# QZ1-boy/CDFO

Hardware: NVIDIA B200
Metric: HR frames/sec, 1080p x4 LD-QP37 (higher is better)
Workload: dtype bf16

## Files before the change

cdfo_b200/_lib.py:

```python
import ctypes
import os
import re
import weakref

import torch

_HERE = os.path.dirname(os.path.abspath(__file__))
SO_PATH = os.path.join(_HERE, "libcdfo_b200.so")

OK = 0
F32, F16, BF16 = 0, 1, 2
_DTYPES = {torch.float32: F32, torch.float16: F16, torch.bfloat16: BF16}


class CdfoError(RuntimeError):
    pass


_lib = None
HEADER = os.path.join(os.path.dirname(_HERE), "include", "cdfo_b200.h")


def _ctype(decl):
    d = decl.strip()
    if "*" in d:
        return ctypes.c_void_p
    base = re.sub(r"\b(const|unsigned|signed)\b", "", d).split()
    t = base[0] if base else "int"
    return {"float": ctypes.c_float, "double": ctypes.c_double, "size_t": ctypes.c_size_t, "int": ctypes.c_int, "int64_t": ctypes.c_int64,
            "uint8_t": ctypes.c_uint8, "long": ctypes.c_long}.get(t, ctypes.c_int)


def prototypes(header=HEADER):
    src = re.sub(r"/\*.*?\*/", "", open(header).read(), flags=re.S)
    src = re.sub(r"//[^\n]*", "", src)
    out = {}
    for ret, name, params in re.findall(r"\b(const\s+char\s*\*|size_t|int|void)\s*(cdfo_[a-z0-9_]+)\s*\(([^)]*)\)\s*;", src, flags=re.S):
        params = " ".join(params.split())
        args = [] if params in ("", "void") else [_ctype(a) for a in params.split(",")]
        res = ctypes.c_char_p if "char" in ret else (ctypes.c_size_t if ret == "size_t" else (None if ret == "void" else ctypes.c_int))
        out[name] = (res, args)
    return out


def _bind_prototypes(handle):
    if not os.path.isfile(HEADER):
        raise CdfoError("cdfo_b200: %s not found (the ctypes prototypes are taken from it)" % HEADER)
    for name, (res, args) in prototypes().items():
        fn = getattr(handle, name, None)
        if fn is None:
            raise CdfoError("cdfo_b200: %s declares %s but %s does not export it (stale build?)" % (HEADER, name, SO_PATH))
        fn.restype, fn.argtypes = res, args


def lib():
    global _lib
    if _lib is None:
        if not os.path.isfile(SO_PATH):
            raise CdfoError(
                "cdfo_b200: %s not found -- build it with `python cdfo_b200/csrc/build.py` "
                "(there is no CPU or PyTorch fallback for this path)" % SO_PATH)
        _lib = ctypes.CDLL(SO_PATH)
        _bind_prototypes(_lib)
    return _lib


_LAUNCHES = {"cdfo_mv_end_fix": 3, "cdfo_lra_fwd": 5, "cdfo_lra_c8_fwd": 5, "cdfo_mdta_fwd": 3, "cdfo_mdta_c8_fwd": 3, "cdfo_psnr_ssim_u8": 3,
             "cdfo_lra_mask_logits_fwd": 2,
             "cdfo_spatial_gate_c8_fwd": 2}
launch_count = 0


def call(name, *args):
    global launch_count
    rc = getattr(lib(), name)(*args)
    if rc != OK:
        check(rc, name)
    launch_count += _LAUNCHES.get(name, 1)
    return rc


def check(rc, what=""):
    if rc != OK:
        msg = lib().cdfo_last_error().decode("utf-8", "replace")
        raise CdfoError("%s failed (status %d): %s" % (what or "cdfo call", rc, msg))


def dtype_code(t: torch.Tensor) -> int:
    try:
        return _DTYPES[t.dtype]
    except KeyError:
        raise CdfoError("cdfo_b200: unsupported dtype %s" % t.dtype)


def ptr(t):
    return ctypes.c_void_p(0 if t is None else t.data_ptr())


def stream_ptr(device=None):
    return ctypes.c_void_p(torch.cuda.current_stream(device).cuda_stream)


def require_cuda(*tensors):
    for t in tensors:
        if t is not None and not t.is_cuda:
            raise NotImplementedError("cdfo_b200 ops are CUDA-only (got a %s tensor)" % t.device)


class TensorCache:

    def __init__(self):
        self._d = {}

    def get(self, t, build, kind=None):
        key = (id(t), kind)
        sig = (t.data_ptr(), str(t.device), t._version, t.dtype)
        hit = self._d.get(key)
        if hit is not None and hit[0]() is t and hit[1] == sig:
            return hit[2]
        val = build()
        d = self._d
        self._d[key] = (weakref.ref(t, lambda _r, k=key: d.pop(k, None)), sig, val)
        return val

    def __len__(self):
        return len(self._d)
```

cdfo_b200/csrc/lra.cu:

```cuda
#include <cuda.h>
#include <cstring>

#include "cdfo_common.cuh"
#include "sm100_ptx.cuh"

namespace cdfo {

__device__ __forceinline__ float warp_max(float v) {
#pragma unroll
  for (int o = 16; o > 0; o >>= 1) v = fmaxf(v, __shfl_xor_sync(0xffffffffu, v, o));
  return v;
}
__device__ __forceinline__ float warp_sum(float v) {
#pragma unroll
  for (int o = 16; o > 0; o >>= 1) v += __shfl_xor_sync(0xffffffffu, v, o);
  return v;
}

__global__ void lra_mask_kernel(const float *__restrict__ u, const float *__restrict__ vmax, const float *__restrict__ qv,
                                uint8_t *__restrict__ midx, float *__restrict__ qsel, int HW) {
  __shared__ float vm[64];
  const int b = blockIdx.y;
  if (threadIdx.x < 64) vm[threadIdx.x] = vmax[b * 64 + threadIdx.x];
  __syncthreads();
// ... 391 lines not shown
  }
}

constexpr int kColWarps = 9, kColThreads = kColWarps * 32;

__global__ void __launch_bounds__(kColThreads, 1) lra_col_kernel(const float *__restrict__ vrow_t, const uint8_t *__restrict__ midx,
                                                                const float *__restrict__ qsel, float *__restrict__ long_out,
                                                                LraTables t, int H, int W) {
  extern __shared__ __align__(16) float sm[];
  const int b = blockIdx.y, w = blockIdx.x;
  const int HW = H * W;
  const int Hk = (H + 63) & ~63;
  float *Q = sm;
  float *V = Q + Hk * kLd;
  float *sq = V;
  const int tid = threadIdx.x, lane = tid & 31, warp = tid >> 5, g = lane >> 2, tq = lane & 3;
  float kh[9];
#pragma unroll
  for (int i = 0; i < 9; ++i) kh[i] = t.kh[i];

  for (int e = tid; e < (H + 8) * 64; e += kColThreads) {
    const int h = (e >> 6) - 4, c = e & 63;
    float v = 0.f;
    if (h >= 0 && h < H) {
      v = t.beta;
      const int cm = midx[(size_t)b * HW + h * W + w];
      if (cm != 255) {
        const int ti = cm - c + 4;
        if (ti >= 0 && ti <= 8) v = fmaf(__ldg(t.kw + ti), qsel[(size_t)b * HW + h * W + w], v);
      }
    }
    sq[e] = v;
  }
  __syncthreads();
  for (int e = tid; e < Hk * 64; e += kColThreads) {
    const int h = e >> 6, c = e & 63;
    float acc = 0.f;
    if (h < H) {
      acc = t.bh;
#pragma unroll
      for (int i = 0; i < 9; ++i) acc = fmaf(kh[i], sq[(h + i) * 64 + c], acc);
    }
    Q[h * kLd + c] = __uint_as_float(to_tf32(acc));
  }
  __syncthreads();
  const float *vsrc = vrow_t + ((size_t)b * W + w) * H * 64;
  for (int e = tid; e < Hk * 16; e += kColThreads) {
    const int r = e >> 4, c4 = (e & 15) * 4;
    float4 v = make_float4(0.f, 0.f, 0.f, 0.f);
    if (r < H) v = *reinterpret_cast<const float4 *>(vsrc + (size_t)r * 64 + c4);
    v.x = __uint_as_float(to_tf32(v.x)); v.y = __uint_as_float(to_tf32(v.y));
    v.z = __uint_as_float(to_tf32(v.z)); v.w = __uint_as_float(to_tf32(v.w));
    *reinterpret_cast<float4 *>(V + r * kLd + c4) = v;
  }
  __syncthreads();

  const uint32_t *Qu = reinterpret_cast<const uint32_t *>(Q), *Vu = reinterpret_cast<const uint32_t *>(V);
  const int n_qt = (H + 15) >> 4, n_kb = Hk >> 6;
  for (int qt = warp; qt < n_qt; qt += kColWarps) {
    const int q0 = qt * 16;
    uint32_t aq[8][4];
#pragma unroll
    for (int s = 0; s < 8; ++s) {
      aq[s][0] = Qu[(q0 + g) * kLd + 8 * s + tq];
      aq[s][1] = Qu[(q0 + g + 8) * kLd + 8 * s + tq];
      aq[s][2] = Qu[(q0 + g) * kLd + 8 * s + tq + 4];
      aq[s][3] = Qu[(q0 + g + 8) * kLd + 8 * s + tq + 4];
    }
    float o[8][4];
#pragma unroll
    for (int n = 0; n < 8; ++n)
#pragma unroll
      for (int i = 0; i < 4; ++i) o[n][i] = 0.f;
    float m_run[2] = {-INFINITY, -INFINITY}, l_run[2] = {0.f, 0.f};
    for (int kb = 0; kb < n_kb; ++kb) {
      const int key0 = kb * 64;
      float sc[8][4];
#pragma unroll
      for (int n = 0; n < 8; ++n) {
#pragma unroll
        for (int i = 0; i < 4; ++i) sc[n][i] = 0.f;
        const uint32_t *kr = Qu + (key0 + 8 * n + g) * kLd + tq;
#pragma unroll
        for (int s = 0; s < 8; ++s) mma_tf32(sc[n], aq[s], kr[8 * s], kr[8 * s + 4]);
      }
      flash_tile_block(sc, m_run, l_run, o, Vu, key0, H, g, tq);
    }
#pragma unroll
    for (int r = 0; r < 2; ++r) {
      l_run[r] += __shfl_xor_sync(0xffffffffu, l_run[r], 1);
      l_run[r] += __shfl_xor_sync(0xffffffffu, l_run[r], 2);
    }
    const float inv0 = 1.f / l_run[0], inv1 = 1.f / l_run[1];
    const int h0 = q0 + g, h1 = q0 + g + 8;
#pragma unroll
    for (int n = 0; n < 8; ++n) {
      if (h0 < H) *reinterpret_cast<float2 *>(long_out + (((size_t)b * H + h0) * W + w) * 64 + 8 * n + 2 * tq) = make_float2(o[n][0] * inv0, o[n][1] * inv0);
      if (h1 < H) *reinterpret_cast<float2 *>(long_out + (((size_t)b * H + h1) * W + w) * 64 + 8 * n + 2 * tq) = make_float2(o[n][2] * inv1, o[n][3] * inv1);
    }
  }
}

constexpr int kQw = 36;

__device__ __forceinline__ void mma_bf16(float (&d)[4], const uint32_t (&a)[4], uint32_t b0, uint32_t b1) {
  asm volatile("mma.sync.aligned.m16n8k16.row.col.f32.bf16.bf16.f32 {%0, %1, %2, %3}, {%4, %5, %6, %7}, {%8, %9}, {%0, %1, %2, %3};"
               : "+f"(d[0]), "+f"(d[1]), "+f"(d[2]), "+f"(d[3])
               : "r"(a[0]), "r"(a[1]), "r"(a[2]), "r"(a[3]), "r"(b0), "r"(b1));
}
__device__ __forceinline__ uint32_t pack_bf16x2(float lo, float hi) {
  __nv_bfloat162 v = __floats2bfloat162_rn(lo, hi);
  return *reinterpret_cast<uint32_t *>(&v);
}

__global__ void __launch_bounds__(kColThreads, 2) lra_col_bf16_kernel(const float *__restrict__ vrow_t, const uint8_t *__restrict__ midx,
                                                                     const float *__restrict__ qsel, float *__restrict__ long_out,
                                                                     LraTables t, int H, int W) {
  extern __shared__ __align__(16) uint32_t smu[];
  const int b = blockIdx.y, w = blockIdx.x;
  const int HW = H * W;
  const int Hk = (H + 63) & ~63;
  const int SW = Hk / 2 + 4;
  uint32_t *Qw = smu;
  uint32_t *Vt = Qw + Hk * kQw;
  float *cq = reinterpret_cast<float *>(Vt + 64 * SW);
  int *cm = reinterpret_cast<int *>(cq + H + 8);
  float *kws = reinterpret_cast<float *>(cm + H + 8);
  const int tid = threadIdx.x, lane = tid & 31, warp = tid >> 5, g = lane >> 2, tq = lane & 3;
  float kh[9];
#pragma unroll
  for (int i = 0; i < 9; ++i) kh[i] = t.kh[i];
  if (tid < 9) kws[tid] = t.kw[tid];
  for (int e = tid; e < H + 8; e += kColThreads) {
    const int h = e - 4;
    int c = -1;
    float q = 0.f;
    if (h >= 0 && h < H) {
      c = midx[(size_t)b * HW + h * W + w];
      q = qsel[(size_t)b * HW + h * W + w];
    }
    cm[e] = c;
    cq[e] = q;
  }
  {
    const float *vsrc = vrow_t + ((size_t)b * W + w) * H * 64;
    for (int e = tid; e < (Hk / 2) * 16; e += kColThreads) {
      const int kp = (e >> 6) * 4 + (e & 3), c4 = (e >> 2) & 15;
      float4 v0 = make_float4(0.f, 0.f, 0.f, 0.f), v1 = v0;
      if (2 * kp < H) v0 = __ldg(reinterpret_cast<const float4 *>(vsrc + (size_t)(2 * kp) * 64 + c4 * 4));
      if (2 * kp + 1 < H) v1 = __ldg(reinterpret_cast<const float4 *>(vsrc + (size_t)(2 * kp + 1) * 64 + c4 * 4));
      const uint32_t wv[4] = {pack_bf16x2(v0.x, v1.x), pack_bf16x2(v0.y, v1.y), pack_bf16x2(v0.z, v1.z), pack_bf16x2(v0.w, v1.w)};
#pragma unroll
      for (int i = 0; i < 4; ++i) {
        const int j = (i + (c4 >> 1)) & 3;
        Vt[(c4 * 4 + j) * SW + kp] = j == 0 ? wv[0] : (j == 1 ? wv[1] : (j == 2 ? wv[2] : wv[3]));
      }
    }
  }
  __syncthreads();
  for (int e = tid; e < Hk * 32; e += kColThreads) {
    const int h = e >> 5, c0 = (e & 31) * 2;
    float a0 = 0.f, a1 = 0.f;
    if (h < H) {
      a0 = a1 = t.bh;
#pragma unroll
      for (int i = 0; i < 9; ++i) {
        const int c = cm[h + i];
        if (c < 0) continue;
        float s0 = t.beta, s1 = t.beta;
        if (c != 255) {
          const int t0 = c - c0 + 4, t1 = t0 - 1;
          const float q = cq[h + i];
          if (t0 >= 0 && t0 <= 8) s0 = fmaf(kws[t0], q, s0);
          if (t1 >= 0 && t1 <= 8) s1 = fmaf(kws[t1], q, s1);
        }
        a0 = fmaf(kh[i], s0, a0);
        a1 = fmaf(kh[i], s1, a1);
      }
    }
    Qw[h * kQw + (e & 31)] = pack_bf16x2(a0, a1);
  }
  __syncthreads();

  const int n_qt = (H + 15) >> 4, n_kb = Hk >> 6;
  for (int qt = warp; qt < n_qt; qt += kColWarps) {
    const int q0 = qt * 16;
    float o[8][4];
#pragma unroll
    for (int n = 0; n < 8; ++n)
#pragma unroll
      for (int i = 0; i < 4; ++i) o[n][i] = 0.f;
    float m_run[2] = {-INFINITY, -INFINITY}, l_run[2] = {0.f, 0.f};
    for (int kb = 0; kb < n_kb; ++kb) {
      const int key0 = kb * 64;
      float sc[8][4];
      {
        uint32_t aq[4][4];
#pragma unroll
        for (int s = 0; s < 4; ++s) {
          aq[s][0] = Qw[(q0 + g) * kQw + 8 * s + tq];
          aq[s][1] = Qw[(q0 + g + 8) * kQw + 8 * s + tq];
          aq[s][2] = Qw[(q0 + g) * kQw + 8 * s + tq + 4];
          aq[s][3] = Qw[(q0 + g + 8) * kQw + 8 * s + tq + 4];
        }
#pragma unroll
        for (int n = 0; n < 8; ++n) {
#pragma unroll
          for (int i = 0; i < 4; ++i) sc[n][i] = 0.f;
          const uint32_t *kr = Qw + (key0 + 8 * n + g) * kQw + tq;
#pragma unroll
          for (int s = 0; s < 4; ++s) mma_bf16(sc[n], aq[s], kr[8 * s], kr[8 * s + 4]);
        }
      }
      float mx[2] = {-INFINITY, -INFINITY};
#pragma unroll
      for (int n = 0; n < 8; ++n) {
        const int key = key0 + 8 * n + 2 * tq;
        if (key >= H) { sc[n][0] = -INFINITY; sc[n][2] = -INFINITY; }
        if (key + 1 >= H) { sc[n][1] = -INFINITY; sc[n][3] = -INFINITY; }
        mx[0] = fmaxf(mx[0], fmaxf(sc[n][0], sc[n][1]));
        mx[1] = fmaxf(mx[1], fmaxf(sc[n][2], sc[n][3]));
      }
      float scale[2];
#pragma unroll
      for (int r = 0; r < 2; ++r) {
        mx[r] = fmaxf(mx[r], __shfl_xor_sync(0xffffffffu, mx[r], 1));
        mx[r] = fmaxf(mx[r], __shfl_xor_sync(0xffffffffu, mx[r], 2));
        const float m_new = fmaxf(m_run[r], mx[r]);
        scale[r] = expf(m_run[r] - m_new);
        m_run[r] = m_new;
        l_run[r] *= scale[r];
      }
#pragma unroll
      for (int n = 0; n < 8; ++n) {
        sc[n][0] = expf(sc[n][0] - m_run[0]); sc[n][1] = expf(sc[n][1] - m_run[0]);
        sc[n][2] = expf(sc[n][2] - m_run[1]); sc[n][3] = expf(sc[n][3] - m_run[1]);
        l_run[0] += sc[n][0] + sc[n][1];
        l_run[1] += sc[n][2] + sc[n][3];
        o[n][0] *= scale[0]; o[n][1] *= scale[0]; o[n][2] *= scale[1]; o[n][3] *= scale[1];
      }
#pragma unroll
      for (int s = 0; s < 4; ++s) {
        const uint32_t ap[4] = {pack_bf16x2(sc[2 * s][0], sc[2 * s][1]), pack_bf16x2(sc[2 * s][2], sc[2 * s][3]),
                                pack_bf16x2(sc[2 * s + 1][0], sc[2 * s + 1][1]), pack_bf16x2(sc[2 * s + 1][2], sc[2 * s + 1][3])};
        const uint32_t *vr = Vt + g * SW + (key0 >> 1) + 8 * s + tq;
#pragma unroll
        for (int n = 0; n < 8; ++n) mma_bf16(o[n], ap, vr[8 * n * SW], vr[8 * n * SW + 4]);
      }
    }
#pragma unroll
    for (int r = 0; r < 2; ++r) {
      l_run[r] += __shfl_xor_sync(0xffffffffu, l_run[r], 1);
      l_run[r] += __shfl_xor_sync(0xffffffffu, l_run[r], 2);
    }
    const float inv0 = 1.f / l_run[0], inv1 = 1.f / l_run[1];
    const int h0 = q0 + g, h1 = q0 + g + 8;
#pragma unroll
    for (int n = 0; n < 8; ++n) {
      if (h0 < H) *reinterpret_cast<float2 *>(long_out + (((size_t)b * H + h0) * W + w) * 64 + 8 * n + 2 * tq) = make_float2(o[n][0] * inv0, o[n][1] * inv0);
      if (h1 < H) *reinterpret_cast<float2 *>(long_out + (((size_t)b * H + h1) * W + w) * 64 + 8 * n + 2 * tq) = make_float2(o[n][2] * inv1, o[n][3] * inv1);
    }
  }
}

constexpr int kWinThreads = 256;
__global__ void __launch_bounds__(kWinThreads) lra_win_kernel(const float *__restrict__ qv, const uint8_t *__restrict__ midx,
                                                             float *__restrict__ loc_out, int H, int W) {
  extern __shared__ __align__(16) float sm[];
  float *q = sm;
  float *v = q + 64 * kLd;
  float *Ps = v + 64 * kLd;
  const int b = blockIdx.z, wy = blockIdx.y, wx = blockIdx.x;
  const int HW = H * W;
  const int tid = threadIdx.x;
  static_assert(kWinThreads == 256, "one token and 16 + 16 channels per thread");
  {
    const int tok = tid & 63, cg = tid >> 6;
    const int h = wy * 8 + (tok >> 3), w = wx * 8 + (tok & 7);
    const size_t pix = (size_t)h * W + w;
    const int cm = midx[(size_t)b * HW + pix];
    const float *qp = qv + ((size_t)b * 128 + cg) * HW + pix;
    float qr[16], vv[16];
#pragma unroll
    for (int k = 0; k < 16; ++k) {
      qr[k] = __ldg(qp + (size_t)(4 * k) * HW);
      vv[k] = __ldg(qp + (size_t)(64 + 4 * k) * HW);
    }
#pragma unroll
    for (int k = 0; k < 16; ++k) {
      const int c = 4 * k + cg;
      q[tok * kLd + c] = cm == c ? 0.f : qr[k];
      v[tok * kLd + c] = vv[k];
    }
  }
  __syncthreads();
  const float *Kcur = q;
  flash_block_fp32_kptr(q, &Kcur, v, Ps, 64, [&](int) {}, [&](int tok, int c4, float4 val) {
    const int h = wy * 8 + (tok >> 3), w = wx * 8 + (tok & 7);
    *reinterpret_cast<float4 *>(loc_out + (((size_t)b * H + h) * W + w) * 64 + c4) = val;
  });
}

constexpr int kWinTcThreads = 128, kWinLd = 36;
__global__ void __launch_bounds__(kWinTcThreads, 6) lra_win_tc_kernel(const float *__restrict__ qv, const uint8_t *__restrict__ midx,
                                                                      float *__restrict__ loc_out, int H, int W) {
  __shared__ uint32_t Qh[64 * kWinLd], Ql[64 * kWinLd], Vt[64 * kWinLd], Vl[64 * kWinLd];
  const int b = blockIdx.z, wy = blockIdx.y, wx = blockIdx.x;
  const int HW = H * W;
  const int tid = threadIdx.x, lane = tid & 31, warp = tid >> 5, g = lane >> 2, tq = lane & 3;
  {
    const int tok = tid & 63, half = tid >> 6;
    const int h = wy * 8 + (tok >> 3), w = wx * 8 + (tok & 7);
    const size_t pix = (size_t)h * W + w;
    const int cm = midx[(size_t)b * HW + pix];
    const float *qp = qv + ((size_t)b * 128 + half * 32) * HW + pix;
#pragma unroll 4
    for (int k = 0; k < 16; ++k) {
      const int c = half * 32 + 2 * k;
      float q0 = __ldg(qp + (size_t)(2 * k) * HW), q1 = __ldg(qp + (size_t)(2 * k + 1) * HW);
      if (cm == c) q0 = 0.f;
      if (cm == c + 1) q1 = 0.f;
      const __nv_bfloat16 h0 = __float2bfloat16_rn(q0), h1 = __float2bfloat16_rn(q1);
      Qh[tok * kWinLd + (c >> 1)] = pack_bf16x2(__bfloat162float(h0), __bfloat162float(h1));
      Ql[tok * kWinLd + (c >> 1)] = pack_bf16x2(q0 - __bfloat162float(h0), q1 - __bfloat162float(h1));
      const float v0 = __ldg(qp + (size_t)(64 + 2 * k) * HW), v1 = __ldg(qp + (size_t)(64 + 2 * k + 1) * HW);
      const __nv_bfloat16 vh0 = __float2bfloat16_rn(v0), vh1 = __float2bfloat16_rn(v1);
      reinterpret_cast<__nv_bfloat16 *>(Vt)[(c * kWinLd) * 2 + tok] = vh0;
      reinterpret_cast<__nv_bfloat16 *>(Vt)[((c + 1) * kWinLd) * 2 + tok] = vh1;
      reinterpret_cast<__nv_bfloat16 *>(Vl)[(c * kWinLd) * 2 + tok] = __float2bfloat16_rn(v0 - __bfloat162float(vh0));
      reinterpret_cast<__nv_bfloat16 *>(Vl)[((c + 1) * kWinLd) * 2 + tok] = __float2bfloat16_rn(v1 - __bfloat162float(vh1));
    }
  }
  __syncthreads();
  const int q0r = warp * 16;
  uint32_t ah[4][4], al[4][4];
#pragma unroll
  for (int s = 0; s < 4; ++s) {
    ah[s][0] = Qh[(q0r + g) * kWinLd + 8 * s + tq];      ah[s][1] = Qh[(q0r + g + 8) * kWinLd + 8 * s + tq];
    ah[s][2] = Qh[(q0r + g) * kWinLd + 8 * s + tq + 4];  ah[s][3] = Qh[(q0r + g + 8) * kWinLd + 8 * s + tq + 4];
    al[s][0] = Ql[(q0r + g) * kWinLd + 8 * s + tq];      al[s][1] = Ql[(q0r + g + 8) * kWinLd + 8 * s + tq];
    al[s][2] = Ql[(q0r + g) * kWinLd + 8 * s + tq + 4];  al[s][3] = Ql[(q0r + g + 8) * kWinLd + 8 * s + tq + 4];
  }
  float sc[8][4];
#pragma unroll
  for (int n = 0; n < 8; ++n) {
#pragma unroll
    for (int i = 0; i < 4; ++i) sc[n][i] = 0.f;
    const uint32_t *kh_ = Qh + (8 * n + g) * kWinLd + tq, *kl_ = Ql + (8 * n + g) * kWinLd + tq;
#pragma unroll
    for (int s = 0; s < 4; ++s) {
      const uint32_t bh0 = kh_[8 * s], bh1 = kh_[8 * s + 4];
      mma_bf16(sc[n], al[s], bh0, bh1);
      mma_bf16(sc[n], ah[s], kl_[8 * s], kl_[8 * s + 4]);
      mma_bf16(sc[n], ah[s], bh0, bh1);
    }
  }
  float mx[2] = {-INFINITY, -INFINITY}, sum[2] = {0.f, 0.f};
#pragma unroll
  for (int n = 0; n < 8; ++n) {
    mx[0] = fmaxf(mx[0], fmaxf(sc[n][0], sc[n][1]));
    mx[1] = fmaxf(mx[1], fmaxf(sc[n][2], sc[n][3]));
  }
#pragma unroll
  for (int r = 0; r < 2; ++r) {
    mx[r] = fmaxf(mx[r], __shfl_xor_sync(0xffffffffu, mx[r], 1));
    mx[r] = fmaxf(mx[r], __shfl_xor_sync(0xffffffffu, mx[r], 2));
  }
#pragma unroll
  for (int n = 0; n < 8; ++n) {
    sc[n][0] = expf(sc[n][0] - mx[0]); sc[n][1] = expf(sc[n][1] - mx[0]);
    sc[n][2] = expf(sc[n][2] - mx[1]); sc[n][3] = expf(sc[n][3] - mx[1]);
    sum[0] += sc[n][0] + sc[n][1];
    sum[1] += sc[n][2] + sc[n][3];
  }
  float o[8][4];
#pragma unroll
  for (int n = 0; n < 8; ++n)
#pragma unroll
    for (int i = 0; i < 4; ++i) o[n][i] = 0.f;
#pragma unroll
  for (int s = 0; s < 4; ++s) {
    uint32_t ap[4], apl[4];
#pragma unroll
    for (int i = 0; i < 4; ++i) {
      const float p0 = sc[2 * s + (i >> 1)][2 * (i & 1)], p1 = sc[2 * s + (i >> 1)][2 * (i & 1) + 1];
      const float h0 = __bfloat162float(__float2bfloat16_rn(p0)), h1 = __bfloat162float(__float2bfloat16_rn(p1));
      ap[i] = pack_bf16x2(h0, h1);
      apl[i] = pack_bf16x2(p0 - h0, p1 - h1);
    }
    const uint32_t *vr = Vt + g * kWinLd + 8 * s + tq, *vl = Vl + g * kWinLd + 8 * s + tq;
#pragma unroll
    for (int n = 0; n < 8; ++n) {
      const uint32_t b0 = vr[8 * n * kWinLd], b1 = vr[8 * n * kWinLd + 4];
      mma_bf16(o[n], apl, b0, b1);
      mma_bf16(o[n], ap, vl[8 * n * kWinLd], vl[8 * n * kWinLd + 4]);
      mma_bf16(o[n], ap, b0, b1);
    }
  }
#pragma unroll
  for (int r = 0; r < 2; ++r) {
    sum[r] += __shfl_xor_sync(0xffffffffu, sum[r], 1);
    sum[r] += __shfl_xor_sync(0xffffffffu, sum[r], 2);
  }
  const float inv0 = 1.f / sum[0], inv1 = 1.f / sum[1];
  const int t0 = q0r + g, t1 = t0 + 8;
  float *d0 = loc_out + (((size_t)b * H + wy * 8 + (t0 >> 3)) * W + wx * 8 + (t0 & 7)) * 64 + 2 * tq;
  float *d1 = loc_out + (((size_t)b * H + wy * 8 + (t1 >> 3)) * W + wx * 8 + (t1 & 7)) * 64 + 2 * tq;
#pragma unroll
  for (int n = 0; n < 8; ++n) {
    *reinterpret_cast<float2 *>(d0 + 8 * n) = make_float2(o[n][0] * inv0, o[n][1] * inv0);
    *reinterpret_cast<float2 *>(d1 + 8 * n) = make_float2(o[n][2] * inv1, o[n][3] * inv1);
  }
}

}

using namespace cdfo;

typedef CUresult (*LraEncodeTiledFn)(CUtensorMap *, CUtensorMapDataType, cuuint32_t, void *, const cuuint64_t *, const cuuint64_t *,
                                     const cuuint32_t *, const cuuint32_t *, CUtensorMapInterleave, CUtensorMapSwizzle,
                                     CUtensorMapL2promotion, CUtensorMapFloatOOBfill);
static LraEncodeTiledFn lra_encode_tiled_fn() {
  static LraEncodeTiledFn fn = nullptr;
  if (!fn) {
    void *ptr = nullptr;
    cudaDriverEntryPointQueryResult q;
    if (cudaGetDriverEntryPoint("cuTensorMapEncodeTiled", &ptr, cudaEnableDefault, &q) == cudaSuccess && q == cudaDriverEntryPointSuccess)
      fn = reinterpret_cast<LraEncodeTiledFn>(ptr);
  }
  return fn;
}

static bool g_lra_row_tma = true;
extern "C" int cdfo_lra_set_row_tma(int on) {
  g_lra_row_tma = on != 0;
  return CDFO_OK;
}
static bool g_lra_col_tf32 = false;
static bool g_lra_col_tc = true;
static bool g_lra_win_tc = true;
extern "C" int cdfo_lra_set_col_precision(int tf32) {
  g_lra_col_tf32 = tf32 != 0;
  return CDFO_OK;
}
extern "C" int cdfo_lra_set_col_tcgen05(int on) {
  g_lra_col_tc = on != 0;
  return CDFO_OK;
}
extern "C" int cdfo_lra_set_win_tensor_core(int on) {
  g_lra_win_tc = on != 0;
  return CDFO_OK;
}

extern "C" size_t cdfo_lra_workspace_bytes(int B, int H, int W) {
  const size_t P = (size_t)B * H * W;
  return P * (1 + 4) + 3 * P * 64 * 4 + 256;
}

static int lra_run(const float *qv, const float *u, const float *vmax, const float *x, const float *x2, const float *tables,
                   float beta, float bh, const float *fuse_w, const float *fuse_b, float *out, void *out_c8, int out_channels,
                   int channel0, void *workspace, int B, int H, int W, void *stream);

extern "C" int cdfo_lra_fwd(const float *qv, const float *u, const float *vmax, const float *x, const float *x2, const float *tables,
                            float beta, float bh, const float *fuse_w, const float *fuse_b, float *out, void *workspace, int B,
                            int H, int W, void *stream) {
  return lra_run(qv, u, vmax, x, x2, tables, beta, bh, fuse_w, fuse_b, out, nullptr, 0, 0, workspace, B, H, W, stream);
}

extern "C" int cdfo_lra_c8_fwd(const float *qv, const float *u, const float *vmax, const float *x, const float *x2, const float *tables,
                               float beta, float bh, const float *fuse_w, const float *fuse_b, void *out_c8, int out_channels,
                               int channel0, void *workspace, int B, int H, int W, void *stream) {
  CDFO_REQUIRE(out_c8 && ((uintptr_t)out_c8 & 15) == 0, CDFO_ERR_NULL, "cdfo_lra_c8_fwd: out_c8 must be a 16-byte aligned pointer");
  CDFO_REQUIRE(out_channels % 8 == 0 && channel0 % 8 == 0 && channel0 >= 0 && channel0 + 64 <= out_channels, CDFO_ERR_SHAPE,
               "cdfo_lra_c8_fwd: channels [%d, %d) do not fit %d output channels (multiples of 8)", channel0, channel0 + 64, out_channels);
  return lra_run(qv, u, vmax, x, x2, tables, beta, bh, fuse_w, fuse_b, nullptr, out_c8, out_channels, channel0, workspace, B, H, W, stream);
}

static int lra_run(const float *qv, const float *u, const float *vmax, const float *x, const float *x2, const float *tables,
                   float beta, float bh, const float *fuse_w, const float *fuse_b, float *out, void *out_c8, int out_channels,
                   int channel0, void *workspace, int B, int H, int W, void *stream) {
  CDFO_REQUIRE(qv && u && vmax && x && tables && fuse_w && fuse_b && (out || out_c8) && workspace, CDFO_ERR_NULL, "cdfo_lra_fwd: NULL pointer");
  CDFO_REQUIRE(B > 0 && B <= 65535 && H > 0 && W > 0 && H % 8 == 0 && W % 8 == 0, CDFO_ERR_SHAPE,
               "cdfo_lra_fwd: H and W must be multiples of the window size 8 (got %d x %d)", H, W);
  cudaStream_t s = (cudaStream_t)stream;
  const size_t P = (size_t)B * H * W;
  const int HW = H * W;
  uint8_t *ws = (uint8_t *)workspace;
  float *qsel = (float *)ws;
  float *vrow_t = qsel + P;
  float *long_out = vrow_t + P * 64;
  float *loc_out = long_out + P * 64;
  uint8_t *midx = (uint8_t *)(loc_out + P * 64);
  LraTables t{tables, tables + 9, tables + 18, tables + 82, beta, bh};

  lra_mask_kernel<<<dim3(ceil_div(HW, 128), B), 128, 0, s>>>(u, vmax, qv, midx, qsel, HW);

  const int Wk = (W + 63) & ~63;
  const size_t row_smem = ((size_t)Wk * kLd + 4096 + 3 * (size_t)Wk + 64 + kRowThreads + 2 * (size_t)Wk) * 4;
  const int Hk = (H + 63) & ~63;
  const size_t col_v = (size_t)Hk * kLd > (size_t)(H + 8) * 64 ? (size_t)Hk * kLd : (size_t)(H + 8) * 64;
  const size_t col_smem = ((size_t)Hk * kLd + col_v) * 4;
  const size_t win_smem = (size_t)3 * 64 * kLd * 4;
  const int kDynMax = 224 * 1024;
  CDFO_REQUIRE(row_smem <= (size_t)kDynMax && col_smem <= (size_t)kDynMax, CDFO_ERR_UNSUPPORTED,
               "cdfo_lra_fwd: frame %d x %d exceeds the shared-memory row/column buffers (W <= 704, H <= 384)", H, W);
  static bool attr = false;
  if (!attr) {
    cudaError_t e1 = cudaFuncSetAttribute(lra_row_kernel<false>, cudaFuncAttributeMaxDynamicSharedMemorySize, kDynMax);
    if (e1 == cudaSuccess) e1 = cudaFuncSetAttribute(lra_row_kernel<true>, cudaFuncAttributeMaxDynamicSharedMemorySize, kDynMax);
    cudaError_t e2 = cudaFuncSetAttribute(lra_col_kernel, cudaFuncAttributeMaxDynamicSharedMemorySize, kDynMax);
    if (e2 == cudaSuccess) e2 = cudaFuncSetAttribute(lra_col_bf16_kernel, cudaFuncAttributeMaxDynamicSharedMemorySize, kDynMax);
    cudaError_t e3 = cudaFuncSetAttribute(lra_win_kernel, cudaFuncAttributeMaxDynamicSharedMemorySize, (int)win_smem);
    if (e1 != cudaSuccess || e2 != cudaSuccess || e3 != cudaSuccess)
      return fail(CDFO_ERR_CUDA, "cdfo_lra_fwd: cudaFuncSetAttribute failed: %s", cudaGetErrorString(e1 != cudaSuccess ? e1 : (e2 != cudaSuccess ? e2 : e3)));
    attr = true;
  }
  {
    CUtensorMap qm;
    memset(&qm, 0, sizeof(qm));
    bool row_tma = g_lra_row_tma && W % 4 == 0 && ((uintptr_t)qv & 15) == 0 && row_smem + kRowRawBytes <= (size_t)kDynMax;
    if (row_tma) {
      static LraEncodeTiledFn enc = lra_encode_tiled_fn();
      if (enc) {
        const cuuint64_t gdim[3] = {(cuuint64_t)W, (cuuint64_t)H, (cuuint64_t)B * 128};
        const cuuint64_t gstr[2] = {(cuuint64_t)W * 4, (cuuint64_t)H * W * 4};
        const cuuint32_t box[3] = {kRowPiece, 1, 64};
        const cuuint32_t estr[3] = {1, 1, 1};
        CUresult cr = enc(&qm, CU_TENSOR_MAP_DATA_TYPE_FLOAT32, 3, const_cast<float *>(qv), gdim, gstr, box, estr, CU_TENSOR_MAP_INTERLEAVE_NONE,
                          CU_TENSOR_MAP_SWIZZLE_NONE, CU_TENSOR_MAP_L2_PROMOTION_L2_128B, CU_TENSOR_MAP_FLOAT_OOB_FILL_NONE);
        CDFO_REQUIRE(cr == CUDA_SUCCESS, CDFO_ERR_CUDA, "cuTensorMapEncodeTiled(qv rows) failed with CUresult %d", (int)cr);
      } else {
        row_tma = false;
      }
    }
    if (row_tma) lra_row_kernel<true><<<dim3(H, B), kRowThreads, row_smem + kRowRawBytes, s>>>(qm, qv, midx, qsel, vrow_t, t, H, W);
    else lra_row_kernel<false><<<dim3(H, B), kRowThreads, row_smem, s>>>(qm, qv, midx, qsel, vrow_t, t, H, W);
  }
  int col_done = 0;
  if (!g_lra_col_tf32 && g_lra_col_tc) {
    col_done = lra_col_sm100_launch(vrow_t, midx, qsel, long_out, t, B, H, W, s);
    if (col_done < 0) return col_done;
  }
  if (col_done) {
  } else if (g_lra_col_tf32) {
    lra_col_kernel<<<dim3(W, B), kColThreads, col_smem, s>>>(vrow_t, midx, qsel, long_out, t, H, W);
  } else {
    const size_t col16_smem = ((size_t)Hk * kQw + 64 * ((size_t)Hk / 2 + 4) + 2 * (size_t)(H + 8) + 16) * 4;
    lra_col_bf16_kernel<<<dim3(W, B), kColThreads, col16_smem, s>>>(vrow_t, midx, qsel, long_out, t, H, W);
  }
  if (g_lra_win_tc) lra_win_tc_kernel<<<dim3(W / 8, H / 8, B), kWinTcThreads, 0, s>>>(qv, midx, loc_out, H, W);
  else lra_win_kernel<<<dim3(W / 8, H / 8, B), kWinThreads, win_smem, s>>>(qv, midx, loc_out, H, W);
  if (int rc = check_launch("cdfo_lra_fwd")) return rc;
  return pointwise_conv(long_out, loc_out, fuse_w, fuse_b, x, x2, out, B, 128, 64, HW, 0, 1, s, out_c8, out_channels, channel0);
}
```

include/cdfo_b200.h:

```cpp
#ifndef CDFO_B200_H_
#define CDFO_B200_H_

#include <stddef.h>
#include <stdint.h>

#ifdef __cplusplus
extern "C" {
#endif

typedef enum cdfo_status {
  CDFO_OK = 0,
  CDFO_ERR_SHAPE = -1,
  CDFO_ERR_NULL = -2,
  CDFO_ERR_CUDA = -3,
  CDFO_ERR_UNSUPPORTED = -4,
  CDFO_ERR_NO_DEVICE = -5
} cdfo_status;

typedef enum cdfo_dtype { CDFO_F32 = 0, CDFO_F16 = 1, CDFO_BF16 = 2 } cdfo_dtype;
#define CDFO_FIELDS_F16X4 16

const char *cdfo_last_error(void);
int cdfo_version(void);
int cdfo_device_ok(int dev);

int cdfo_dcn_fwd(const void *x, const void *offset, const void *mask, const void *weight,
                 const void *bias, void *y, int B, int C, int H, int W, int Co, int kh, int kw,
                 int stride_h, int stride_w, int pad_h, int pad_w, int dil_h, int dil_w,
                 int groups, int dg, int dtype, void *stream);

int cdfo_dcn_sample_index(const float *offset, int32_t *idx, int B, int H, int W, int kh, int kw,
                          int stride_h, int stride_w, int pad_h, int pad_w, int dil_h, int dil_w,
                          int dg, void *stream);

int cdfo_flow_warp_fwd(const float *x, const float *flow, float *y, int B, int C, int H, int W,
                       int32_t *idx, void *stream);

int cdfo_mv2mvs(const void *mv, int mv_is_int32, float *flows, int H, int W, void *stream);
int cdfo_mv2mvs_ra(const void *mv_l0, const void *mv_l1, int mv_is_int32, float *flows, int H, int W, void *stream);
int cdfo_mv_end_fix(float *flows, int B, int H, int W, int i, int max_idx, void *stream);

int cdfo_prior_conv_fwd(const float *x, const float *w, const float *bias, float *y, int B, int Co, int H, int W, void *stream);
int cdfo_prior_conv_act_fwd(const float *x, const float *w, const float *bias, float *y, int B, int Co, int H, int W, int relu, void *stream);

int cdfo_pack_c8(const float *x_nchw, void *x_c8, int B, int C, int H, int W, void *stream);
int cdfo_pack_c8_into(const float *x_nchw, void *x_c8, int B, int C, int H, int W, int out_channels, int channel0, void *stream);
int cdfo_unpack_c8(const void *x_c8, float *x_nchw, int B, int C, int H, int W, void *stream);

int cdfo_dcn_sm100_fwd(const void *x_q4p, const void *offset, const void *mask, const float *mv,
                       const void *wpk, const float *bias, void *y, int B, int H, int W, int dg,
                       int off_dtype, int out_mode, int num_ctas, int x_batch, long long off_bstride,
                       long long msk_bstride, void *stream);
int cdfo_dcn_sm100_pack_weight(const float *w, void *wpk, void *stream);
int cdfo_pack_q4p(const float *x_nchw, void *x_q4p, int B, int C, int H, int W, void *stream);
int cdfo_dcn_tex_sm100_fwd(const void *x_q4t, const void *fields, const float *mv, const void *wpk, const float *bias,
                           void *y, int B, int H, int W, int dg, int out_mode, int num_ctas, int x_batch,
                           long long fields_bstride, void *stream);
int cdfo_dcn_tex_sm100_set_fields_path(int use_tma);
int cdfo_dcn_tex_sm100_stacked_fwd(const void *x_q4t, const void *fields, const float *mv, const void *wpk, const float *bias,
                                   void *y_stack, int n_seq, int n_groups, int stack_chunks, const int *group_chunk, int H,
                                   int W, int dg, int x_batch, void *stream);
int cdfo_dcn_tex_sm100_pack_weight(const float *w, void *wpk, void *stream);
int cdfo_mv_head_dcn_fused_sm100_fwd(const void *z_c8, const void *head_wpk, const float *head_bias, float magnitude,
                                     const void *x_q4t, const float *mv, const void *dcn_wpk, const float *dcn_bias, void *y,
                                     void *fields_out, int B, int H, int W, int out_mode, int x_batch, int num_ctas, void *stream);
int cdfo_mv_head_dcn_fused_sm100_stacked_fwd(const void *z_c8, const void *head_wpk, const float *head_bias, float magnitude,
                                             const void *x_q4t, const float *mv, const void *dcn_wpk, const float *dcn_bias,
                                             void *y_stack, int n_seq, int n_groups, int stack_chunks, const int *group_chunk,
                                             int H, int W, int x_batch, void *stream);
int cdfo_pack_q4t(const float *x_nchw, void *x_q4t, int B, int C, int H, int W, void *stream);
int cdfo_q4t_pitch(int W);
size_t cdfo_q4t_bytes(int B, int C, int H, int W);
int cdfo_conv3x3_sm100_fwd(const void *x_c8, const void *wpk, const float *bias, const void *resid_c8, void *y,
                           int B, int Cin, int Cout, int H, int W, int act, int out_mode, void *stream);
int cdfo_mv_offset_head_sm100_fwd(const void *z_c8, const void *wpk, const float *bias, const void *first, void *out,
                                  int B, int Cin, int dg, int H, int W, float magnitude, void *stream);
int cdfo_mv_offset_head_dual_sm100_fwd(const void *z_c8, const void *wpk, const float *bias, void *out, int B, int Cin, int dg, int H,
                                       int W, float magnitude, void *stream);
int cdfo_conv_last_skip_sm100_fwd(const void *x_c8, const void *wpk, const float *bias, const float *lr, float *y, int B,
                                  int Cin, int H, int W, void *stream);
int cdfo_conv3x3_sm100_pack_weight(const float *w, void *wpk, int Cout, int Cin, void *stream);
int cdfo_conv_sm100_fwd(const void *x_c8, const void *wpk, const float *bias, const void *resid_c8, void *y, int B, int Cin,
                        int Cout, int H, int W, int ksize, int act, int out_mode, void *stream);
int cdfo_conv_sm100_pack_weight(const float *w, void *wpk, int Cout, int Cin, int ksize, void *stream);
size_t cdfo_conv_sm100_weight_bytes(int Cout, int Cin, int ksize);
size_t cdfo_conv3x3_sm100_weight_bytes(int Cout, int Cin);
int cdfo_conv3x3_sm100_ntile(int Cout, int Cin);
int cdfo_mdta_fwd(const float *x, int x_batch, const float *extra, const float *pred, const float *flow,
                  const float *fusion_w, const float *du_w1, const float *du_b1, const float *du_w2, const float *du_b2,
                  const float *temperature, const float *proj_w, int heads, int mode, void *out, float *ca_sums,
                  void *workspace, int B, int H, int W, void *stream);
int cdfo_mdta_c8_fwd(const void *x_c8, int x_batch, const void *extra_c8, const void *pred_c8, const float *flow, const float *fusion_w,
                     const float *du_w1, const float *du_b1, const float *du_w2, const float *du_b2, const float *temperature,
                     const float *proj_w, int heads, void *out_c8, void *workspace, int B, int H, int W, void *stream);
size_t cdfo_mdta_workspace_bytes(int B, int H, int W, int heads);
int cdfo_mdta_parts(int B);
int cdfo_channel_gate_fwd(const float *partial_sums, int parts, const float *w1, const float *b1, const float *w2,
                          const float *b2, float *gate, int B, int C, int Cmid, int HW, void *stream);
int cdfo_pack_c8_scaled(const float *x_nchw, const float *scale, void *x_c8, int B, int C, int H, int W, void *stream);
int cdfo_unpack_c8_add(const void *x_c8, const float *add_nchw, int add_batch, float *y_nchw, int B, int C, int H, int W,
                       void *stream);
int cdfo_resample_c8(const void *a, const void *b, const void *base, void *y, int B, int C, int Ho, int Wo, int mode, void *stream);
int cdfo_lra_fwd(const float *qv, const float *u, const float *vmax, const float *x, const float *x2, const float *tables,
                 float beta, float bh, const float *fuse_w, const float *fuse_b, float *out, void *workspace, int B, int H, int W,
                 void *stream);
int cdfo_lra_set_col_precision(int tf32);
int cdfo_lra_set_col_tcgen05(int on);
int cdfo_lra_set_win_tensor_core(int on);
int cdfo_lra_set_row_tma(int on);
int cdfo_lra_c8_fwd(const float *qv, const float *u, const float *vmax, const float *x, const float *x2, const float *tables,
                    float beta, float bh, const float *fuse_w, const float *fuse_b, void *out_c8, int out_channels, int channel0,
                    void *workspace, int B, int H, int W, void *stream);
int cdfo_pointwise_conv_fwd(const float *in1, const float *in2, const float *w, const float *bias, const float *resid1,
                            const float *resid2, float *out, int B, int K, int Co, int H, int W, int act, int mode, void *stream);
int cdfo_pointwise_conv_c8_fwd(const float *in1, const float *in2, const float *w, const float *bias, const float *resid1,
                               const float *resid2, void *out_c8, int B, int K, int Co, int H, int W, int act, int mode,
                               int out_channels, int channel0, void *stream);
size_t cdfo_lra_workspace_bytes(int B, int H, int W);
int cdfo_layernorm_c_fwd(const void *x, const float *gamma, const float *beta, void *y, int B, int C, int H, int W, float eps,
                         int dtype, void *stream);
int cdfo_dwconv3x3_fwd(const void *x, const float *w, void *y, int B, int C, int H, int W, int dtype, void *stream);
int cdfo_mdta_gram_fwd(const void *qk, float *partial, int B, int Ctot, int H, int W, int parts, int dtype, void *stream);
int cdfo_conv3x3_pair_sm100_supported(int Cout, int Cin);
size_t cdfo_conv3x3_pair_sm100_weight_bytes(int Cout, int Cin);
int cdfo_conv3x3_pair_sm100_pack_weight(const float *w, void *wpk, int Cout, int Cin, void *stream);
int cdfo_conv3x3_pair_sm100_fwd(const void *x_c8, const void *wpk, const float *bias, const void *resid_c8, void *y_c8, int B, int Cin,
                                int Cout, int H, int W, int act, void *stream);
int cdfo_conv3x3_pair_sm100_planes_fwd(const void *x_c8, const void *wpk, const float *bias, const void *resid_c8, void *y, int B,
                                       int Cin, int Cout, int H, int W, int act, int y_planes, void *stream);
int cdfo_conv3x3_pair_sm100_edge_fwd(const void *x_c8, const void *wpk, const float *bias, const float *bias_edge, const void *resid_c8,
                                     void *y, int B, int Cin, int Cout, int H, int W, int act, int y_planes, void *stream);
int cdfo_conv4x4s2_pair_sm100_supported(int Cout, int Cin);
size_t cdfo_conv4x4s2_pair_sm100_weight_bytes(int Cin);
int cdfo_conv4x4s2_pair_sm100_pack_weight(const float *w3, void *wpk, int Cin, void *stream);
int cdfo_conv4x4s2_pair_sm100_fwd(const void *x_c8, const void *wpk, const float *bias, const void *resid_c8, void *y_c8, int B, int Cin,
                                  int H_in, int W_in, void *stream);
int cdfo_conv4x4s2_pair_sm100_planes_fwd(const void *x, const void *wpk, const float *bias, const void *resid_c8, void *y_c8, int B,
                                         int Cin, int H_in, int W_in, int x_planes, void *stream);
int cdfo_conv4x4s2_pair_sm100_block_fwd(const void *x, const void *wpk, const float *bias, const void *resid_c8, const void *up_c8,
                                        void *y_c8, void *half_c8, int B, int Cin, int H_in, int W_in, int x_planes, void *stream);
int cdfo_planes_to_unit_f32(const void *src, int src_kind, float *dst, int n_planes, int H_in, int W, int H_out, void *stream);
int cdfo_sr_to_u8(const float *sr, uint8_t *out, int n_planes, int H_in, int W, int H_out, void *stream);
size_t cdfo_psnr_ssim_workspace_bytes(int B, int H, int W, int border);
int cdfo_psnr_ssim_u8(const uint8_t *res, const uint8_t *gt, int B, int H, int W, int border, double *frame_out, double *accum,
                      void *workspace, void *stream);
int cdfo_umma_selftest(const void *A, const void *B, float *D, int swap_lbo_sbo, void *stream);

size_t cdfo_lra_mask_logits_workspace_bytes(int B, int H, int W);
int cdfo_lra_mask_logits_fwd(const float *v, const float *w2, const float *b2, const float *w3, const float *b3, float *vmax,
                             void *workspace, int B, int H, int W, void *stream);
int cdfo_lra_set_logit_tma(int on);

int cdfo_prior_conv_c8_fwd(const float *x, const float *w, const float *bias, void *y_c8, int B, int Co, int H, int W, int lrelu, void *stream);
int cdfo_layernorm_c8_fwd(const void *x_c8, const float *gamma, const float *beta, void *y_c8, int B, int H, int W, float eps, void *stream);
int cdfo_dwconv3x3_c8_fwd(const void *x_c8, const float *w, void *y_c8, int B, int C, int H, int W, void *stream);
int cdfo_mdta_gram_c8_fwd(const void *qkv_c8, float *partial, int B, int C, int H, int W, int parts, void *stream);
int cdfo_mdta_fold_fwd(const float *partial, const float *temperature, const float *project_out, float *M, int B, int parts, void *stream);
int cdfo_mdta_apply_c8_fwd(const void *qkv_c8, int C, int v_channel0, const float *M, const void *x1_c8, const void *x2_c8, void *out1_c8,
                           void *out2_c8, int B, int H, int W, void *stream);
int cdfo_conv16_c8_fwd(const void *x_c8, const float *w, const float *bias, void *y_c8, int B, int Hi, int Wi, int Ho, int Wo, int y_channels,
                       int transposed, void *stream);
int cdfo_spatial_gate_c8_fwd(const void *x_c8, const float *w, const float *bias, void *pooled_ws, void *y_c8, int B, int H, int W, void *stream);

#ifdef __cplusplus
}
#endif
#endif
```

Before: 86.84.

## Fuse LRA window attention with the output fuse projection in a persistent kernel

New measurement: 85.92, median of 6. 1.1% lower.

```diff
diff --git a/cdfo_b200/_lib.py b/cdfo_b200/_lib.py
--- a/cdfo_b200/_lib.py
+++ b/cdfo_b200/_lib.py
@@ -65,7 +65,7 @@
     return _lib
 
 
-_LAUNCHES = {"cdfo_mv_end_fix": 3, "cdfo_lra_fwd": 5, "cdfo_lra_c8_fwd": 5, "cdfo_mdta_fwd": 3, "cdfo_mdta_c8_fwd": 3, "cdfo_psnr_ssim_u8": 3,
+_LAUNCHES = {"cdfo_mv_end_fix": 3, "cdfo_lra_fwd": 4, "cdfo_lra_c8_fwd": 4, "cdfo_mdta_fwd": 3, "cdfo_mdta_c8_fwd": 3, "cdfo_psnr_ssim_u8": 3,
              "cdfo_lra_mask_logits_fwd": 2,
              "cdfo_spatial_gate_c8_fwd": 2}
 launch_count = 0
diff --git a/cdfo_b200/csrc/lra.cu b/cdfo_b200/csrc/lra.cu
--- a/cdfo_b200/csrc/lra.cu
+++ b/cdfo_b200/csrc/lra.cu
@@ -717,10 +717,12 @@
 }
 
 constexpr int kWinTcThreads = 128, kWinLd = 36;
-__global__ void __launch_bounds__(kWinTcThreads, 6) lra_win_tc_kernel(const float *__restrict__ qv, const uint8_t *__restrict__ midx,
-                                                                      float *__restrict__ loc_out, int H, int W) {
-  __shared__ uint32_t Qh[64 * kWinLd], Ql[64 * kWinLd], Vt[64 * kWinLd], Vl[64 * kWinLd];
-  const int b = blockIdx.z, wy = blockIdx.y, wx = blockIdx.x;
+constexpr int kWinTcWords = 4 * 64 * kWinLd;
+
+template <int LOAD_UNROLL>
+__device__ __forceinline__ void win_tc_attention(const float *__restrict__ qv, const uint8_t *__restrict__ midx, uint32_t *S, int b, int wy,
+                                                 int wx, int H, int W, float (&o)[8][4], float (&inv)[2]) {
+  uint32_t *Qh = S, *Ql = S + 64 * kWinLd, *Vt = S + 2 * 64 * kWinLd, *Vl = S + 3 * 64 * kWinLd;
   const int HW = H * W;
   const int tid = threadIdx.x, lane = tid & 31, warp = tid >> 5, g = lane >> 2, tq = lane & 3;
   {
@@ -729,7 +731,7 @@
     const size_t pix = (size_t)h * W + w;
     const int cm = midx[(size_t)b * HW + pix];
     const float *qp = qv + ((size_t)b * 128 + half * 32) * HW + pix;
-#pragma unroll 4
+#pragma unroll LOAD_UNROLL
     for (int k = 0; k < 16; ++k) {
       const int c = half * 32 + 2 * k;
       float q0 = __ldg(qp + (size_t)(2 * k) * HW), q1 = __ldg(qp + (size_t)(2 * k + 1) * HW);
@@ -788,7 +790,6 @@
     sum[0] += sc[n][0] + sc[n][1];
     sum[1] += sc[n][2] + sc[n][3];
   }
-  float o[8][4];
 #pragma unroll
   for (int n = 0; n < 8; ++n)
 #pragma unroll
@@ -817,14 +818,157 @@
     sum[r] += __shfl_xor_sync(0xffffffffu, sum[r], 1);
     sum[r] += __shfl_xor_sync(0xffffffffu, sum[r], 2);
   }
-  const float inv0 = 1.f / sum[0], inv1 = 1.f / sum[1];
-  const int t0 = q0r + g, t1 = t0 + 8;
+  inv[0] = 1.f / sum[0];
+  inv[1] = 1.f / sum[1];
+}
+
+__global__ void __launch_bounds__(kWinTcThreads, 6) lra_win_tc_kernel(const float *__restrict__ qv, const uint8_t *__restrict__ midx,
+                                                                      float *__restrict__ loc_out, int H, int W) {
+  __shared__ __align__(16) uint32_t S[kWinTcWords];
+  const int b = blockIdx.z, wy = blockIdx.y, wx = blockIdx.x;
+  const int lane = threadIdx.x & 31, warp = threadIdx.x >> 5, g = lane >> 2, tq = lane & 3;
+  float o[8][4], inv[2];
+  win_tc_attention<4>(qv, midx, S, b, wy, wx, H, W, o, inv);
+  const int t0 = warp * 16 + g, t1 = t0 + 8;
   float *d0 = loc_out + (((size_t)b * H + wy * 8 + (t0 >> 3)) * W + wx * 8 + (t0 & 7)) * 64 + 2 * tq;
   float *d1 = loc_out + (((size_t)b * H + wy * 8 + (t1 >> 3)) * W + wx * 8 + (t1 & 7)) * 64 + 2 * tq;
 #pragma unroll
   for (int n = 0; n < 8; ++n) {
-    *reinterpret_cast<float2 *>(d0 + 8 * n) = make_float2(o[n][0] * inv0, o[n][1] * inv0);
-    *reinterpret_cast<float2 *>(d1 + 8 * n) = make_float2(o[n][2] * inv1, o[n][3] * inv1);
+    *reinterpret_cast<float2 *>(d0 + 8 * n) = make_float2(o[n][0] * inv[0], o[n][1] * inv[0]);
+    *reinterpret_cast<float2 *>(d1 + 8 * n) = make_float2(o[n][2] * inv[1], o[n][3] * inv[1]);
+  }
+}
+
+constexpr int kFuseLdW = 132;
+constexpr int kWinFuseDynSmem = 64 * kFuseLdW * 4;
+constexpr int kWinFuseCtasPerSM = 3;
+constexpr int kStageLd = 68;
+static_assert(4 * 16 * kStageLd <= 2 * 64 * kWinLd, "the four warps' output staging fits over Qh and Ql");
+
+__device__ __forceinline__ void prefetch_l2(const void *p) { asm volatile("prefetch.global.L2 [%0];" ::"l"(p)); }
+
+__device__ __forceinline__ void prefetch_win_fuse(const float *qv, const uint8_t *midx, const float *long_out, const float *x, const float *x2,
+                                                  int b, int wy, int wx, int H, int W) {
+  const int HW = H * W, tid = threadIdx.x;
+  const size_t px0 = (size_t)(wy * 8) * W + wx * 8;
+  for (int e = tid; e < 128 * 8; e += kWinTcThreads)
+    prefetch_l2(qv + ((size_t)b * 128 + (e >> 3)) * HW + px0 + (size_t)(e & 7) * W);
+  for (int e = tid; e < 64 * 8; e += kWinTcThreads) {
+    const size_t off = ((size_t)b * 64 + (e >> 3)) * HW + px0 + (size_t)(e & 7) * W;
+    prefetch_l2(x + off);
+    if (x2) prefetch_l2(x2 + off);
+  }
+  {
+    const int px = tid >> 1;
+    prefetch_l2(long_out + ((size_t)b * HW + px0 + (size_t)(px >> 3) * W + (px & 7)) * 64 + (tid & 1) * 32);
+    if (tid < 8) prefetch_l2(midx + (size_t)b * HW + px0 + (size_t)tid * W);
+  }
+}
+
+__global__ void __launch_bounds__(kWinTcThreads, kWinFuseCtasPerSM)
+    lra_win_fuse_kernel(const float *__restrict__ qv, const uint8_t *__restrict__ midx, const float *__restrict__ long_out,
+                        const float *__restrict__ fuse_w, const float *__restrict__ fuse_b, const float *__restrict__ x,
+                        const float *__restrict__ x2, float *__restrict__ out, uint4 *__restrict__ out8, int out_chunks, int chunk0, int B,
+                        int H, int W) {
+  __shared__ __align__(16) uint32_t S[kWinTcWords];
+  extern __shared__ __align__(16) uint32_t Wf[];
+  const int tid = threadIdx.x, lane = tid & 31, warp = tid >> 5, g = lane >> 2, tq = lane & 3;
+  const int HW = H * W, nwx = W >> 3, nwy = H >> 3, nwin = B * nwy * nwx;
+  if (blockIdx.x < nwin) prefetch_win_fuse(qv, midx, long_out, x, x2, blockIdx.x / (nwx * nwy), (blockIdx.x / nwx) % nwy, blockIdx.x % nwx, H, W);
+  for (int e = tid; e < 64 * 128; e += kWinTcThreads) Wf[(e >> 7) * kFuseLdW + (e & 127)] = to_tf32(__ldg(fuse_w + e));
+  const int src_lo = (lane & ~3) | (tq >> 1), src_hi = src_lo + 2;
+  const bool odd = tq & 1;
+  for (int win = blockIdx.x; win < nwin; win += gridDim.x) {
+    const int wx = win % nwx, wy = (win / nwx) % nwy, b = win / (nwx * nwy);
+    const int next = win + gridDim.x;
+    if (next < nwin) prefetch_win_fuse(qv, midx, long_out, x, x2, next / (nwx * nwy), (next / nwx) % nwy, next % nwx, H, W);
+    __syncthreads();
+    float o[8][4], inv[2];
+    win_tc_attention<16>(qv, midx, S, b, wy, wx, H, W, o, inv);
+
+    const size_t row0 = (size_t)(wy * 8 + 2 * warp) * W + wx * 8;
+    const float *lp = long_out + ((size_t)b * HW + row0 + g) * 64 + tq;
+    float acc[4][2][4];
+#pragma unroll
+    for (int m = 0; m < 4; ++m)
+#pragma unroll
+      for (int n = 0; n < 2; ++n)
+#pragma unroll
+        for (int i = 0; i < 4; ++i) acc[m][n][i] = 0.f;
+#pragma unroll
+    for (int k0 = 0; k0 < 128; k0 += 8) {
+      uint32_t bf[2][2];
+      if (k0 < 64) {
+#pragma unroll
+        for (int n = 0; n < 2; ++n) {
+          bf[n][0] = to_tf32(__ldg(lp + (size_t)n * W * 64 + k0));
+          bf[n][1] = to_tf32(__ldg(lp + (size_t)n * W * 64 + k0 + 4));
+        }
+      } else {
+        const int j = (k0 - 64) >> 3;
+#pragma unroll
+        for (int n = 0; n < 2; ++n) {
+          const float l0 = o[j][2 * n] * inv[n], l1 = o[j][2 * n + 1] * inv[n];
+          const float a0 = __shfl_sync(0xffffffffu, l0, src_lo), a1 = __shfl_sync(0xffffffffu, l1, src_lo);
+          const float c0 = __shfl_sync(0xffffffffu, l0, src_hi), c1 = __shfl_sync(0xffffffffu, l1, src_hi);
+          bf[n][0] = to_tf32(odd ? a1 : a0);
+          bf[n][1] = to_tf32(odd ? c1 : c0);
+        }
+      }
+#pragma unroll
+      for (int m = 0; m < 4; ++m) {
+        const uint32_t *wr = Wf + (m * 16 + g) * kFuseLdW + k0 + tq;
+        const uint32_t af[4] = {wr[0], wr[8 * kFuseLdW], wr[4], wr[8 * kFuseLdW + 4]};
+        mma_tf32(acc[m][0], af, bf[0][0], bf[0][1]);
+        mma_tf32(acc[m][1], af, bf[1][0], bf[1][1]);
+      }
+    }
+#pragma unroll
+    for (int m = 0; m < 4; ++m)
+#pragma unroll
+      for (int r = 0; r < 2; ++r) {
+        const int co = m * 16 + g + 8 * r;
+        const float bb = __ldg(fuse_b + co);
+#pragma unroll
+        for (int n = 0; n < 2; ++n) {
+          const size_t oi = ((size_t)b * 64 + co) * HW + row0 + (size_t)n * W + 2 * tq;
+          float2 v = make_float2(acc[m][n][2 * r] + bb, acc[m][n][2 * r + 1] + bb);
+          const float2 r1 = __ldg(reinterpret_cast<const float2 *>(x + oi));
+          v.x += r1.x; v.y += r1.y;
+          if (x2) {
+            const float2 r2 = __ldg(reinterpret_cast<const float2 *>(x2 + oi));
+            v.x += r2.x; v.y += r2.y;
+          }
+          if (out8) {
+            acc[m][n][2 * r] = v.x;
+            acc[m][n][2 * r + 1] = v.y;
+          } else {
+            *reinterpret_cast<float2 *>(out + oi) = v;
+          }
+        }
+      }
+    if (out8) {
+      __syncthreads();
+      float *stage = reinterpret_cast<float *>(S) + warp * 16 * kStageLd;
+#pragma unroll
+      for (int m = 0; m < 4; ++m)
+#pragma unroll
+        for (int r = 0; r < 2; ++r)
+#pragma unroll
+          for (int n = 0; n < 2; ++n) {
+            stage[(8 * n + 2 * tq) * kStageLd + m * 16 + g + 8 * r] = acc[m][n][2 * r];
+            stage[(8 * n + 2 * tq + 1) * kStageLd + m * 16 + g + 8 * r] = acc[m][n][2 * r + 1];
+          }
+      __syncwarp();
+#pragma unroll
+      for (int i = 0; i < 4; ++i) {
+        const int e = lane + 32 * i, px = e & 15, c8 = e >> 4;
+        const float4 lo = *reinterpret_cast<const float4 *>(stage + px * kStageLd + 8 * c8);
+        const float4 hi = *reinterpret_cast<const float4 *>(stage + px * kStageLd + 8 * c8 + 4);
+        out8[((size_t)b * out_chunks + chunk0 + c8) * HW + row0 + (size_t)(px >> 3) * W + (px & 7)] =
+            make_uint4(pack_bf16x2(lo.x, lo.y), pack_bf16x2(lo.z, lo.w), pack_bf16x2(hi.x, hi.y), pack_bf16x2(hi.z, hi.w));
+      }
+    }
   }
 }
 
@@ -854,6 +998,7 @@
 static bool g_lra_col_tf32 = false;
 static bool g_lra_col_tc = true;
 static bool g_lra_win_tc = true;
+static bool g_lra_win_fuse = true;
 extern "C" int cdfo_lra_set_col_precision(int tf32) {
   g_lra_col_tf32 = tf32 != 0;
   return CDFO_OK;
@@ -866,10 +1011,14 @@
   g_lra_win_tc = on != 0;
   return CDFO_OK;
 }
+extern "C" int cdfo_lra_set_win_fuse(int on) {
+  g_lra_win_fuse = on != 0;
+  return CDFO_OK;
+}
 
 extern "C" size_t cdfo_lra_workspace_bytes(int B, int H, int W) {
   const size_t P = (size_t)B * H * W;
-  return P * (1 + 4) + 3 * P * 64 * 4 + 256;
+  return P * (1 + 4) + 2 * P * 64 * 4 + 256;
 }
 
 static int lra_run(const float *qv, const float *u, const float *vmax, const float *x, const float *x2, const float *tables,
@@ -895,6 +1044,7 @@
                    float beta, float bh, const float *fuse_w, const float *fuse_b, float *out, void *out_c8, int out_channels,
                    int channel0, void *workspace, int B, int H, int W, void *stream) {
   CDFO_REQUIRE(qv && u && vmax && x && tables && fuse_w && fuse_b && (out || out_c8) && workspace, CDFO_ERR_NULL, "cdfo_lra_fwd: NULL pointer");
+  CDFO_REQUIRE((((uintptr_t)x | (uintptr_t)x2 | (uintptr_t)out) & 15) == 0, CDFO_ERR_SHAPE, "cdfo_lra_fwd: x, x2 and out must be 16-byte aligned");
   CDFO_REQUIRE(B > 0 && B <= 65535 && H > 0 && W > 0 && H % 8 == 0 && W % 8 == 0, CDFO_ERR_SHAPE,
                "cdfo_lra_fwd: H and W must be multiples of the window size 8 (got %d x %d)", H, W);
   cudaStream_t s = (cudaStream_t)stream;
@@ -904,8 +1054,7 @@
   float *qsel = (float *)ws;
   float *vrow_t = qsel + P;
   float *long_out = vrow_t + P * 64;
-  float *loc_out = long_out + P * 64;
-  uint8_t *midx = (uint8_t *)(loc_out + P * 64);
+  uint8_t *midx = (uint8_t *)(long_out + P * 64);
   LraTables t{tables, tables + 9, tables + 18, tables + 82, beta, bh};
 
   lra_mask_kernel<<<dim3(ceil_div(HW, 128), B), 128, 0, s>>>(u, vmax, qv, midx, qsel, HW);
@@ -926,6 +1075,7 @@
     cudaError_t e2 = cudaFuncSetAttribute(lra_col_kernel, cudaFuncAttributeMaxDynamicSharedMemorySize, kDynMax);
     if (e2 == cudaSuccess) e2 = cudaFuncSetAttribute(lra_col_bf16_kernel, cudaFuncAttributeMaxDynamicSharedMemorySize, kDynMax);
     cudaError_t e3 = cudaFuncSetAttribute(lra_win_kernel, cudaFuncAttributeMaxDynamicSharedMemorySize, (int)win_smem);
+    if (e3 == cudaSuccess) e3 = cudaFuncSetAttribute(lra_win_fuse_kernel, cudaFuncAttributeMaxDynamicSharedMemorySize, kWinFuseDynSmem);
     if (e1 != cudaSuccess || e2 != cudaSuccess || e3 != cudaSuccess)
       return fail(CDFO_ERR_CUDA, "cdfo_lra_fwd: cudaFuncSetAttribute failed: %s", cudaGetErrorString(e1 != cudaSuccess ? e1 : (e2 != cudaSuccess ? e2 : e3)));
     attr = true;
@@ -963,6 +1113,14 @@
     const size_t col16_smem = ((size_t)Hk * kQw + 64 * ((size_t)Hk / 2 + 4) + 2 * (size_t)(H + 8) + 16) * 4;
     lra_col_bf16_kernel<<<dim3(W, B), kColThreads, col16_smem, s>>>(vrow_t, midx, qsel, long_out, t, H, W);
   }
+  if (g_lra_win_fuse && g_lra_win_tc) {
+    const int nwin = B * (H / 8) * (W / 8);
+    const int grid = nwin < kWinFuseCtasPerSM * kNumSMs ? nwin : kWinFuseCtasPerSM * kNumSMs;
+    lra_win_fuse_kernel<<<grid, kWinTcThreads, kWinFuseDynSmem, s>>>(qv, midx, long_out, fuse_w, fuse_b, x, x2, out, (uint4 *)out_c8,
+                                                                      out_channels / 8, channel0 / 8, B, H, W);
+    return check_launch("cdfo_lra_fwd");
+  }
+  float *loc_out = vrow_t;
   if (g_lra_win_tc) lra_win_tc_kernel<<<dim3(W / 8, H / 8, B), kWinTcThreads, 0, s>>>(qv, midx, loc_out, H, W);
   else lra_win_kernel<<<dim3(W / 8, H / 8, B), kWinThreads, win_smem, s>>>(qv, midx, loc_out, H, W);
   if (int rc = check_launch("cdfo_lra_fwd")) return rc;
diff --git a/include/cdfo_b200.h b/include/cdfo_b200.h
--- a/include/cdfo_b200.h
+++ b/include/cdfo_b200.h
@@ -107,6 +107,7 @@
 int cdfo_lra_set_col_precision(int tf32);
 int cdfo_lra_set_col_tcgen05(int on);
 int cdfo_lra_set_win_tensor_core(int on);
+int cdfo_lra_set_win_fuse(int on);
 int cdfo_lra_set_row_tma(int on);
 int cdfo_lra_c8_fwd(const float *qv, const float *u, const float *vmax, const float *x, const float *x2, const float *tables,
                     float beta, float bh, const float *fuse_w, const float *fuse_b, void *out_c8, int out_channels, int channel0,
```
